# lmmontoya-ai/taboo-brittleness

Measured on AMD Instinct MI355X. Metric: prompts/sec SAE-ablation sweep Gemma-2-9B @L32, higher is better.
Workload: dtype bf16

## Files before the change

taboo_brittleness_amd/csrc/api.h:

```cpp
#pragma once
#include <hip/hip_runtime.h>
#include <stdint.h>

void tb_rmsnorm(const uint16_t* x, const uint16_t* w, uint16_t* y, int M, int D, float eps, hipStream_t st);
void tb_add_rmsnorm2(uint16_t* h, const uint16_t* o, const uint16_t* w_post, const uint16_t* w_next, uint16_t* x,
                     int M, int D, float eps, hipStream_t st);
void tb_embed_rmsnorm(const int32_t* ids, const uint16_t* E, const uint16_t* w, uint16_t* h, uint16_t* x, int M,
                      int D, int V, float scale, float eps, hipStream_t st);
void tb_rope_qkv_cache(const uint16_t* qkv, const int32_t* pos, const int32_t* slot_of_row, const float* cos_t,
                       const float* sin_t, uint16_t* q_out, uint16_t* kc, uint16_t* vc, int M, int Hq, int Hkv,
                       int HD, int S, int max_pos, hipStream_t st);
void tb_rope_qkv_cache_part(const float* part, int ks, const int32_t* pos, const int32_t* slot_of_row,
                            const float* cos_t, const float* sin_t, uint16_t* q_out, uint16_t* kc, uint16_t* vc, int M,
                            int Hq, int Hkv, int HD, int S, int max_pos, hipStream_t st);
void tb_kv_fanout(uint16_t* kc, uint16_t* vc, const int32_t* src_row, const int32_t* slot, const int32_t* pos, int M,
                  int nlayers, int slots, int Hkv, int S, int HD, hipStream_t st);
int tb_attention_lds_bytes(int HD);
int tb_attention_split_rows(int n, bool prefix);
void tb_attention(const uint16_t* q, const uint16_t* kc, const uint16_t* vc, uint16_t* out, const int32_t* pos,
                  const int32_t* slot, int B, int T, int Hq, int Hkv, int HD, int S, float scale, float softcap,
                  int window, hipStream_t st, const uint16_t* pkc = nullptr, const uint16_t* pvc = nullptr,
                  const int32_t* pslot = nullptr, const int32_t* plen = nullptr);
void tb_attention_varlen(const uint16_t* q, const uint16_t* kc, const uint16_t* vc, uint16_t* out, const int32_t* pos,
                         const int32_t* blk, int nblk, int Hq, int Hkv, int HD, int S, float scale, float softcap,
// ... 8 lines not shown
                    int B, int T, int V, int accumulate, int round_bf16, const int32_t* offs, float* cum,
                    const int32_t* rowmap, hipStream_t st);
int tb_topk_chunks(int R, int V);
void tb_topk_rows(const float* x, float* vals, int32_t* idx, int R, int V, int K, float* wv, int32_t* wi, int C,
                  hipStream_t st);
void tb_xent_rows(const uint16_t* logits, const int32_t* tgt, float* nll, int R, int V, float cap, int emulate_bf16,
                  hipStream_t st);
void tb_register_softcap_table(float cap, const uint16_t* tab);
void tb_decode_head(const uint16_t* logits, const int32_t* tgt, int32_t* nxt, float* nll_self, float* nll_tgt, int R,
                    int V, float cap, hipStream_t st);
bool tb_decode_head_stats(const uint16_t* logits, const int32_t* tgt, int off, float* stats, int R, int V, float cap,
                          hipStream_t st);
void tb_head_merge(const float* part, int npart, const int32_t* tgt, const float* tgt_logit, int32_t* nxt,
                   float* nll_self, float* nll_tgt, float* lse, int M, int V, hipStream_t st);
void tb_head_fused4(const uint16_t* A, const uint16_t* W, float* part, float cap, const int32_t* tgt,
                    float* tgt_logit, int32_t* nxt, float* nll_self, float* nll_tgt, int M, int N, int K, hipStream_t st);
void tb_gemm4_qkv_rope(const uint16_t* A, const uint16_t* W, const int32_t* pos, const int32_t* slot_of_row,
                       const uint16_t* cs, uint16_t* q_out, uint16_t* kc, uint16_t* vc, int M, int K,
                       int Hq, int Hkv, int S, int max_pos, int tile_rows, hipStream_t st, const uint16_t* a2 = nullptr,
                       int k0 = 0);
bool tb_register_softcap_compact(float cap, const uint16_t* tab, int lo, int hi, float sat);
bool tb_softcap_compact(const uint16_t* x, float* y, int n, float cap, hipStream_t st);
bool tb_gemm4_ok(int M, int N, int K);
int tb_gemm4_splitk_ks(int M, int N, int K, int tile_rows);
int tb_gemm4_splitk_part(const uint16_t* A, const uint16_t* W, float* ws, int M, int N, int K, int tile_rows, int ks,
                         hipStream_t st);
void tb_add_rmsnorm2_part(uint16_t* h, const float* part, int ks, const uint16_t* w_post, const uint16_t* w_next,
                          uint16_t* x, int M, int D, float eps, hipStream_t st);
void tb_gemm4_splitk(const uint16_t* A, const uint16_t* W, uint16_t* out, float* ws, int M, int N, int K, int ldo,
                     int epi, int tile_rows, int ks, hipStream_t st);
void tb_row_combine(const int64_t* ptr, const float* coef, float* out, int B, int T, int V, hipStream_t st);
bool tb_random_basis_ok(int D);
void tb_random_basis(const uint64_t* seeds, const int32_t* ranks, const int64_t* rows, int n, int D, float* table,
                     hipStream_t st, int qu = 1);
void tb_gemm4(const uint16_t* A, const uint16_t* W, void* C, const float* bias, const float* thr, int M, int N, int K,
              int ldc, int epi, int tile_rows, hipStream_t st, const uint16_t* a2 = nullptr, int k0 = 0);
void tb_gemm_nt(const uint16_t* A, const uint16_t* W, void* C, const float* bias, const float* thr, int M, int N,
                int K, int ldc, int epi, hipStream_t st);
void tb_lowrank_edit(uint16_t* h, uint16_t* x_next, const uint8_t* apply, const int32_t* idx, const int32_t* cnt,
                     int mmax, const void* E, const void* Dm, int table_f32, const float* bias, const float* thr,
                     const float* pre_bias, float alpha, const uint16_t* w_next, float eps, int M, int D,
                     float* coef_out, hipStream_t st, const float* val = nullptr);
void tb_sae_splice_edit(uint16_t* h, uint16_t* x_next, const uint8_t* apply, const int32_t* src_row,
                        const float* acts, int n_act_rows, int L, const int32_t* idx, const int32_t* cnt, int mmax,
                        const void* Wdec, int table_f32, const float* b_dec, float alpha, const uint16_t* w_next,
                        float eps, int M, int D, hipStream_t st);
// ... 61 lines not shown
```

taboo_brittleness_amd/csrc/bindings.cpp:

```cpp
#include <torch/extension.h>
#include <ATen/hip/impl/HIPStreamMasqueradingAsCUDA.h>
#include <c10/core/DeviceGuard.h>

#include <cstdlib>

#include "api.h"

namespace {

hipStream_t cur_stream() { return c10::hip::getCurrentHIPStreamMasqueradingAsCUDA().stream(); }

#define CHECK_DEV(t) TORCH_CHECK((t).is_cuda(), #t " must be a GPU tensor")
#define CHECK_CONTIG(t) TORCH_CHECK((t).is_contiguous(), #t " must be contiguous")
#define CHECK_BF16(t) TORCH_CHECK((t).scalar_type() == at::kBFloat16, #t " must be bfloat16")
#define CHECK_F32(t) TORCH_CHECK((t).scalar_type() == at::kFloat, #t " must be float32")
#define CHECK_I32(t) TORCH_CHECK((t).scalar_type() == at::kInt, #t " must be int32")
#define CHECK_U8(t) TORCH_CHECK((t).scalar_type() == at::kByte || (t).scalar_type() == at::kBool, #t " must be uint8/bool")
#define IN_BF16(t) CHECK_DEV(t); CHECK_CONTIG(t); CHECK_BF16(t)
#define IN_F32(t) CHECK_DEV(t); CHECK_CONTIG(t); CHECK_F32(t)
#define IN_I32(t) CHECK_DEV(t); CHECK_CONTIG(t); CHECK_I32(t)
#define IN_U8(t) CHECK_DEV(t); CHECK_CONTIG(t); CHECK_U8(t)

bool debug_checks() {
  static const bool on = [] {
// ... 369 lines not shown

void gemm4(torch::Tensor A, torch::Tensor W, torch::Tensor C, c10::optional<torch::Tensor> bias,
           c10::optional<torch::Tensor> thr, int64_t epi, int64_t tile_rows) {
  IN_BF16(A); IN_BF16(W); CHECK_DEV(C); CHECK_CONTIG(C);
  TORCH_CHECK(W.dim() == 2, "gemm4: W must be [N, K]");
  TORCH_CHECK(tile_rows == 256 || tile_rows == 128, "gemm4: tile_rows must be 256 or 128");
  const int K = A.size(-1), M = A.numel() / K, N = W.size(0);
  TORCH_CHECK(W.size(1) == K, "gemm4: K mismatch");
  TORCH_CHECK(tb_gemm4_ok(M, N, K), "gemm4: need N % 256 == 0, K % 64 == 0, K >= 64");
  TORCH_CHECK(epi >= 0 && epi <= 3, "gemm4: epi must be 0..3");
  const int64_t ncols = epi == 3 ? N / 2 : N;
  TORCH_CHECK(C.numel() == (int64_t)M * ncols, "gemm4: C shape");
  TORCH_CHECK(C.scalar_type() == ((epi == 0 || epi == 3) ? at::kBFloat16 : at::kFloat), "gemm4: C dtype");
  if (epi == 2) {
    TORCH_CHECK(!bias.has_value() || !bias->defined() || bias->numel() == N, "gemm4: bias numel must be N");
    TORCH_CHECK(!thr.has_value() || !thr->defined() || thr->numel() == N, "gemm4: thr numel must be N");
  }
  c10::DeviceGuard g(A.device());
  tb_gemm4(cbf(A), cbf(W), C.data_ptr(), epi == 2 ? optf(bias) : nullptr, epi == 2 ? optf(thr) : nullptr, M, N, K,
           (int)ncols, (int)epi, (int)tile_rows, cur_stream());
}

bool gemm4_ok(int64_t M, int64_t N, int64_t K) { return tb_gemm4_ok(M, N, K); }

void gemm_ring(torch::Tensor A, torch::Tensor W, torch::Tensor C, int64_t epi, int64_t bm, int64_t bn, int64_t var) {
  IN_BF16(A); IN_BF16(W); IN_BF16(C);
  TORCH_CHECK(W.dim() == 2, "gemm_ring: W must be [N, K]");
  const int K = A.size(-1), M = A.numel() / K, N = W.size(0);
  TORCH_CHECK(W.size(1) == K, "gemm_ring: K mismatch");
  TORCH_CHECK(epi == 0 || epi == 3, "gemm_ring: epi must be 0 or 3");
  TORCH_CHECK(tb_gemm_ring_ok(M, N, K, (int)epi, (int)bm, (int)bn, (int)var), "gemm_ring: unsupported tile / shape");
  const int64_t ncols = epi == 3 ? N / 2 : N;
  TORCH_CHECK(C.numel() == (int64_t)M * ncols, "gemm_ring: C shape");
  c10::DeviceGuard g(A.device());
  tb_gemm_ring(cbf(A), cbf(W), bf(C), M, N, K, (int)ncols, (int)epi, (int)bm, (int)bn, (int)var, cur_stream());
}

bool gemm_ring_ok(int64_t M, int64_t N, int64_t K, int64_t epi, int64_t bm, int64_t bn, int64_t var) {
  return tb_gemm_ring_ok(M, N, K, (int)epi, (int)bm, (int)bn, (int)var);
}

std::vector<std::pair<int64_t, int64_t>> gemm_ring_tiles(int64_t epi) {
  int bm[64], bn[64];
  const int n = std::min(64, tb_gemm_ring_tiles((int)epi, bm, bn, 64));
  std::vector<std::pair<int64_t, int64_t>> out;
  for (int i = 0; i < n; ++i) out.emplace_back(bm[i], bn[i]);
// ... 660 lines not shown
  m.def("row_gather", &row_gather);
  m.def("share_group", &share_group);
  m.def("share_group_max_rows", &share_group_max_rows);
  m.def("attention_split_rows", [](int64_t n, bool prefix) { return (int64_t)tb_attention_split_rows((int)n, prefix); });
  m.def("attention", &attention);
  m.def("attention_prefix", &attention_prefix);
  m.def("attention_varlen", &attention_varlen);
  m.def("attention_varlen_prefix", &attention_varlen_prefix);
  m.def("geglu", &geglu);
  m.def("argmax_rows", &argmax_rows);
  m.def("row_lse", &row_lse);
  m.def("gather_probs", &gather_probs);
  m.def("lens_colsum", &lens_colsum);
  m.def("topk_rows", &topk_rows);
  m.def("xent_rows", &xent_rows);
  m.def("decode_head", &decode_head);
  m.def("decode_head_stats", &decode_head_stats);
  m.def("register_softcap_table", &register_softcap_table);
  m.def("register_softcap_compact", &register_softcap_compact);
  m.def("softcap_compact", &softcap_compact);
  m.def("gemm_nt", &gemm_nt);
  m.def("gemm4", &gemm4);
  m.def("gemm4_ok", &gemm4_ok);
  m.def("gemm_ring", &gemm_ring);
  m.def("gemm_ring_ok", &gemm_ring_ok);
  m.def("gemm_ring_tiles", &gemm_ring_tiles);
  m.def("gemm_ring_qkv_rope", &gemm_ring_qkv_rope);
  m.def("gemm4_splitk", &gemm4_splitk);
  m.def("gemm4_splitk_ks", &gemm4_splitk_ks);
  m.def("gemm4_splitk_part", &gemm4_splitk_part);
  m.def("add_rmsnorm2_part", &add_rmsnorm2_part);
  m.def("gemm4_qkv_rope", &gemm4_qkv_rope);
  m.def("gemm4_l2a", &gemm4_l2a);
  m.def("gemm_ring_l2a", &gemm_ring_l2a);
  m.def("gemm4_qkv_rope_l2a", &gemm4_qkv_rope_l2a);
  m.def("gemm_ring_qkv_rope_l2a", &gemm_ring_qkv_rope_l2a);
  m.def("lora_t", &lora_t);
  m.def("lora_t_chunks", &lora_t_chunks);
  m.def("row_combine", &row_combine);
  m.def("random_basis", &random_basis);
  m.def("lora_t_ok", &lora_t_ok);
  m.def("head_fused", &head_fused);
  m.def("lens_gemm", &lens_gemm);
  m.def("lowrank_edit", &lowrank_edit);
  m.def("latent_affine_edit", &latent_affine_edit);
  m.def("sae_decode_sparse", &sae_decode_sparse);
// ... 21 lines not shown
```

taboo_brittleness_amd/csrc/gemm4.hip:

```cpp
#include "common.h"
#include "api.h"
#include <algorithm>
#include <cstdlib>
#include <utility>

namespace {

constexpr int G4_THREADS = 256, G4_BN = 256;
constexpr int G4_GROUP_M = 4;
constexpr int G4_SLACK1 = 4;
constexpr int G4_SLACK2 = 0;
#ifndef G4_CNT
#define G4_CNT 1
#endif

typedef __attribute__((address_space(3))) void g4_lds_t;
typedef uint32_t u32x2 __attribute__((ext_vector_type(2)));
typedef __attribute__((address_space(3))) char g4_lds_char;

template <int N>
__device__ __forceinline__ void g4_vmcnt() {
  static_assert(N >= 0 && N < 64, "vmcnt range");
  asm volatile("s_waitcnt vmcnt(%0)" ::"n"(N) : "memory");
}
// ... 42 lines not shown

enum { G4_BF16 = 0, G4_F32 = 1, G4_JUMPRELU = 2, G4_GEGLU = 3, G4_ROPE = 4, G4_HEAD = 5, G4_LENS = 6 };

struct G4Rope {
  const int32_t* pos;
  const int32_t* slot;
  const uint16_t* cs;
  uint16_t* q_out;
  uint16_t* kc;
  uint16_t* vc;
  int Hq, Hkv, S, max_pos;
  const uint16_t* ctab;
  int clo, chi;
  float csat, crc, ccap;
  const int32_t* tgt;
  float* tgt_logit;
  float* part;
  int ksplit, kchunk;
  const uint16_t* a2;
  int k0;
};
constexpr int G4_CTAB_N = 32768;

template <int BM, int EPI, bool L2A = false>
__global__ void __launch_bounds__(G4_THREADS, 1)
gemm4_kernel(const uint16_t* __restrict__ A, const uint16_t* __restrict__ W, void* __restrict__ C,
             const float* __restrict__ bias, const float* __restrict__ thr, int M, int N, int K, int ldc, G4Rope rp) {
#if defined(__HIP_DEVICE_COMPILE__)
  static_assert(BM == 256 || BM == 128 || (BM == 64 && EPI == G4_F32), "tile rows (64: the split-K decode tile)");
  constexpr bool G4C = G4_CNT && BM == 256;
  constexpr int WN = 8, WM = BM / 32;
  constexpr int PIMG = G4_BN * 128, QIMG = BM * 128, STG = PIMG + QIMG;
  constexpr int PI = G4_BN / 32, QI = BM / 32, GL = PI + QI;
  constexpr bool LEPI = EPI == G4_BF16 || EPI == G4_LENS;
  constexpr int RB = EPI == G4_GEGLU ? 128 : 256, ECH = RB / 16, ERPI = 64 / ECH;
  constexpr bool SPARE = LEPI;
  constexpr int EXB = SPARE ? 32768 : 0;
  constexpr int ERR = SPARE ? EXB / (4 * RB) : EPI == G4_GEGLU ? BM / 2 : BM / 4;
  constexpr int ENR = LEPI ? (BM / 2) / ERPI : 1;
  constexpr int CTB = EPI == G4_HEAD ? 4096 : 0;
  static_assert(2 * STG + CTB + EXB <= 160 * 1024, "LDS");
  __shared__ __attribute__((aligned(1024))) char smem[2 * STG + CTB + EXB];

  const int nbn = N / G4_BN, nbm = (M + BM - 1) / BM, nwg = nbn * nbm;
  const int NT = K >> 6, KS = EPI == G4_F32 && rp.ksplit > 1 ? rp.ksplit : 1, KC = KS > 1 ? rp.kchunk : NT;
  const int nwgv = nwg * KS;
#define G4_TILE(v, m0_, n0_)                                                                              \
  do {                                                                                                    \
    const int q_ = nwgv / 8, r_ = nwgv % 8, x_ = (v) % 8;                                                 \
    int b_ = (x_ < r_ ? x_ * (q_ + 1) : r_ * (q_ + 1) + (x_ - r_) * q_) + (v) / 8;                        \
    sk = b_ / nwg;                                                                                        \
    b_ -= sk * nwg;                                                                                       \
// ... 17 lines not shown
  for (int i = 0; i < PI; ++i) vp[i] = (uint32_t)((8 * (4 * i + wid) + (lane >> 3)) * K + lchunk * 8) * 2u;
  int mrows, abytes, abytes2 = 0, nt;
  void *wtile, *atile, *atile2 = nullptr;
#define G4_DESC()                                                                                 \
  do {                                                                                            \
    mrows = min(BM, M - m0);                                                                      \
    wtile = (void*)(W + (size_t)n0 * K + sk * KC * 64);                                           \
    atile = (void*)(A + (size_t)m0 * KA + sk * KC * 64);                                          \
    nt = min(KC, NT - sk * KC);                                                                   \
    abytes = mrows * KA * 2;                                                                      \
    int ln_ = __builtin_amdgcn_mbcnt_hi(~0u, __builtin_amdgcn_mbcnt_lo(~0u, 0u));    \
    asm volatile("" : "+v"(ln_));                                                                 \
    const int lc_ = (ln_ & 7) ^ ((4 * wid + (ln_ >> 4)) & 7);                                     \
    _Pragma("unroll") for (int i = 0; i < QI; ++i)                                                \
      vq[i] = (uint32_t)(min(8 * (4 * i + wid) + (ln_ >> 3), mrows - 1) * KA + lc_ * 8) * 2u;     \
    if constexpr (L2A) {                                                                          \
      atile2 = (void*)(rp.a2 + (size_t)m0 * K2);                                                  \
      abytes2 = mrows * K2 * 2;                                                                   \
      _Pragma("unroll") for (int i = 0; i < QI; ++i)                                              \
        vq2[L2A ? i : 0] = (uint32_t)(min(8 * (4 * i + wid) + (ln_ >> 3), mrows - 1) * K2 + lc_ * 8) * 2u; \
    }                                                                                             \
  } while (0)
  G4_DESC();

  const int xr = (lane & 15) >> 1;
  const int co0 = ((lane >> 4) ^ xr) << 4, co1 = ((4 + (lane >> 4)) ^ xr) << 4;
  constexpr bool RP = EPI == G4_ROPE;
  const int offp = (wn * (RP ? 64 : 128) + (lane & 15)) * 128;
#define G4_PROW(i) (RP ? (((i) >> 2) * 128 + ((i) & 3) * 16) : (i) * 16)
  const int offq = PIMG + (wm * (BM / 2) + (lane & 15)) * 128;

  f32x4 acc[WN][WM];
#pragma unroll
  for (int i = 0; i < WN; ++i)
#pragma unroll
    for (int j = 0; j < WM; ++j) acc[i][j] = (f32x4){0.f, 0.f, 0.f, 0.f};
  bf16x8 p0[WN], q0[WM], p1[WN], q1[WM];

  auto frag = [&](int stg, int off) {
    return __builtin_bit_cast(bf16x8, *reinterpret_cast<const uint4*>(smem + stg * STG + off));
  };
#define G4_STAGE_ONE(g, t, stg)                                                                                    \
  do {                                                                                                             \
    char* d_ = smem + (stg) * STG + wid * 1024;                                                                    \
    if ((g) < PI)                                                                                                  \
      __builtin_amdgcn_raw_ptr_buffer_load_lds(__builtin_amdgcn_make_buffer_rsrc(wtile, 0, wbytes, 0x00020000),    \
                                               (g4_lds_t*)(d_ + (g) * 4096), 16, vp[(g) < PI ? (g) : 0], (t) * 128, 0, 0); \
    else if constexpr (L2A) {                 \
      const bool s2_ = (t) >= NT0;                                                                                 \
      __builtin_amdgcn_raw_ptr_buffer_load_lds(                                                                    \
          __builtin_amdgcn_make_buffer_rsrc(s2_ ? atile2 : atile, 0, s2_ ? abytes2 : abytes, 0x00020000),          \
          (g4_lds_t*)(d_ + PIMG + ((g) - PI) * 4096), 16,                                                          \
          s2_ ? vq2[(g) >= PI ? (g) - PI : 0] : vq[(g) >= PI ? (g) - PI : 0], s2_ ? ((t) - NT0) * 128 : (t) * 128,  \
          0, 0);                                                                                                   \
    } else                                                                                                         \
      __builtin_amdgcn_raw_ptr_buffer_load_lds(__builtin_amdgcn_make_buffer_rsrc(atile, 0, abytes, 0x00020000),    \
                                               (g4_lds_t*)(d_ + PIMG + ((g) - PI) * 4096), 16,                      \
                                               vq[(g) >= PI ? (g) - PI : 0], (t) * 128, 0, 0);                      \
  } while (0)
#define G4_STAGE(t, stg) _Pragma("unroll") for (int g_ = 0; g_ < GL; ++g_) G4_STAGE_ONE(g_, t, stg)
#define G4_MFMA(i, j, pc, qc) asm volatile("v_mfma_f32_16x16x32_bf16 %0, %1, %2, %0" : "+a"(acc[i][j]) : "v"(pc[i]), "v"(qc[j]))
#define G4_MF(u)                                                          \
  do {                                                                    \
    if ((u) < NMF) G4_MFMA((u) / WM, (u) % WM, p0, q0);                   \
    else G4_MFMA(((u) - NMF) / WM, ((u) - NMF) % WM, p1, q1);             \
  } while (0)
  constexpr int NR = WN + WM, NMF = WN * WM, NT2 = 2 * NMF;
  constexpr int BAR1 = NR + G4_SLACK1;
  constexpr int BAR2 = NT2 - NR - G4_SLACK2;
  constexpr int GSP = (NT2 - BAR1) / GL;
  constexpr int N2S = (BAR2 - BAR1) / GSP < GL ? (BAR2 - BAR1) / GSP : GL;
  constexpr int N2 = N2S;
  static_assert(GSP >= 1 && BAR1 < NMF && BAR1 < BAR2, "schedule");
  static_assert(NR - 2 <= 15 && BAR1 >= NR, "lgkmcnt range");
#define G4_PK(i) (G4_PROW(i) / 16)
#define G4_QK(j) (PIMG / 2048 + (j))
#define G4_WAIT()                                                        \
  do {                                                                   \
    if (G4C) asm volatile("s_waitcnt lgkmcnt(%0)" ::"n"(NR - 2));     \
  } while (0)
  const uint32_t lds0 = (uint32_t)(uintptr_t)((g4_lds_char*)smem);
  const uint32_t bp0 = lds0 + offp + co0, bp1 = lds0 + offp + co1;
  const uint32_t bq0 = lds0 + offq - PIMG + co0, bq1 = lds0 + offq - PIMG + co1;

  if constexpr (EPI == G4_HEAD) {
    if (rp.ctab != nullptr) {
      uint16_t* lt = reinterpret_cast<uint16_t*>(smem + 2 * STG);
      for (int i = tid; i < rp.chi - rp.clo; i += G4_THREADS) lt[i] = rp.ctab[i];
    }
    __syncthreads();
  }
  G4_STAGE(0, 0);
  G4_STAGE(min(1, nt - 1), 1);
  bool first_tile = true;
  for (;;) {
  if (first_tile || !LEPI) g4_vmcnt<GL>();
  else g4_vmcnt<GL + ENR>();
  first_tile = false;
  g4_bar();
  if (G4C) {
    asm volatile("s_waitcnt lgkmcnt(0)" ::: "memory");
    g4_rd(p0[0], bp0, G4_PK(0));
#pragma unroll
    for (int j = 0; j < WM; ++j) g4_rd(q0[j], bq0, G4_QK(j));
#pragma unroll
    for (int i = 1; i < WN; ++i) g4_rd(p0[i], bp0, G4_PK(i));
  } else {
#pragma unroll
    for (int i = 0; i < WN; ++i) p0[i] = frag(0, offp + G4_PROW(i) * 128 + co0);
#pragma unroll
    for (int j = 0; j < WM; ++j) q0[j] = frag(0, offq + j * 2048 + co0);
  }

#define G4_POST(u)                                                                              \
  do {                                                                                          \
    if ((u) == BAR2) {                                                                          \
      __builtin_amdgcn_s_waitcnt(g4_vmcnt_enc(N2));                                             \
      g4_bar();                                                                                 \
    }                                                                                           \
    G4_MF(u);                                                                                   \
    const int v_ = (u) - BAR2;                                                                  \
    if (v_ >= 0 && v_ < NR) {                                                                   \
      if (G4C) {                                                                             \
        const uint32_t o_ = (sb ^ 1) * STG;                                                     \
        if (v_ == 0) g4_rd(p0[0], bp0 + o_, G4_PK(0));                                          \
        else if (v_ <= WM) g4_rd(q0[v_ >= 1 && v_ <= WM ? v_ - 1 : 0], bq0 + o_, G4_QK(v_ - 1)); \
        else g4_rd(p0[v_ > WM && v_ < NR ? v_ - WM : 0], bp0 + o_, G4_PK(v_ - WM));             \
      } else if (v_ < WN) p0[v_ >= 0 && v_ < WN ? v_ : 0] = frag(sb ^ 1, offp + G4_PROW(v_) * 128 + co0); \
      else q0[v_ >= WN && v_ < NR ? v_ - WN : 0] = frag(sb ^ 1, offq + (v_ - WN) * 2048 + co0); \
    }                                                                                           \
  } while (0)

  for (int t = 0; t < nt; ++t) {
    const int sb = t & 1, tn = min(t + 2, nt - 1);
#pragma unroll
    for (int u = 0; u < NR; ++u) {
      G4_WAIT();
      G4_MF(u);
      if (G4C) {
        if (u < WN) g4_rd(p1[u < WN ? u : 0], bp1 + sb * STG, G4_PK(u));
        else g4_rd(q1[u >= WN ? u - WN : 0], bq1 + sb * STG, G4_QK(u - WN));
      } else if (u < WN) p1[u < WN ? u : 0] = frag(sb, offp + G4_PROW(u) * 128 + co1);
      else q1[u >= WN ? u - WN : 0] = frag(sb, offq + (u - WN) * 2048 + co1);
    }
#pragma unroll
    for (int u = NR; u < BAR1; ++u) {
      G4_WAIT();
      G4_MF(u);
    }
    __builtin_amdgcn_s_waitcnt(0xc07f);
    g4_bar();
#pragma unroll
    for (int g = 0; g < GL; ++g) {
#pragma unroll
      for (int k = 0; k < GSP; ++k) G4_POST(BAR1 + g * GSP + k);
      G4_STAGE_ONE(g, tn, sb);
    }
#pragma unroll
    for (int u = BAR1 + GL * GSP; u < NT2; ++u) G4_POST(u);
    if (!G4C) asm volatile("s_waitcnt lgkmcnt(0)" ::: "memory");
    __builtin_amdgcn_sched_barrier(0);
  }
  if (G4C) asm volatile("s_waitcnt lgkmcnt(0)" ::: "memory");
#undef G4_WAIT
#undef G4_POST
#undef G4_MF
#undef G4_MFMA
  g4_vmcnt<0>();
  g4_bar();
  const int em0 = m0, en0 = n0, esk = sk;
  const int next = tile + (int)gridDim.x;
  if constexpr (LEPI) {
    if (next < nwgv) {
      tile = next;
      G4_TILE(tile, m0, n0);
      G4_DESC();
      G4_STAGE(0, 0);
      if constexpr (SPARE) G4_STAGE(min(1, nt - 1), 1);
    }
    asm volatile("s_nop 15\n\ts_nop 15" ::: "memory");
    const uint32_t reg = (uint32_t)(uintptr_t)((g4_lds_char*)smem) + (SPARE ? 2 * STG + CTB : STG) + wid * ERR * RB;
    uint16_t* obase = reinterpret_cast<uint16_t*>(C) + (size_t)(em0 + wm * (BM / 2)) * ldc;
    const int nrow = min(BM / 2, M - em0 - wm * (BM / 2));
    const auto ors = __builtin_amdgcn_make_buffer_rsrc(obase, 0, nrow > 0 ? nrow * ldc * 2 : 0, 0x00020000);
    int ln = __builtin_amdgcn_mbcnt_hi(~0u, __builtin_amdgcn_mbcnt_lo(~0u, 0u));
    asm volatile("" : "+v"(ln));
    const int oc0 = (EPI == G4_GEGLU ? (en0 >> 1) + wn * 64 : en0 + wn * 128) + (ln % ECH) * 8;
    constexpr int NI = EPI == G4_GEGLU ? WN / 2 : WN, NRA = ECH / ERPI;
    uint32_t wa[NI], ra[NRA];
#pragma unroll
    for (int i = 0; i < NI; ++i) {
      const int cb = 32 * i + 8 * (ln >> 4);
      wa[i] = reg + (ln & 15) * RB + (((cb >> 4) ^ (ln & 15 & (ECH - 1))) << 4) + (cb & 15);
    }
// ... 224 lines not shown
      const int n = nb + i * 16;
      float4 bn_ = make_float4(0.f, 0.f, 0.f, 0.f), th = bn_;
      if constexpr (EPI == G4_JUMPRELU) {
        if (bias) bn_ = *reinterpret_cast<const float4*>(bias + n);
        if (thr) th = *reinterpret_cast<const float4*>(thr + n);
      }
#pragma unroll
      for (int j = 0; j < WM; ++j) {
        const int m = mb + j * 16;
        if (m >= M) continue;
        const f32x4 v = acc[i][j];
        if constexpr (EPI == G4_F32) {
          *reinterpret_cast<float4*>(reinterpret_cast<float*>(C) + ((size_t)esk * M + m) * ldc + n) =
              make_float4(v[0], v[1], v[2], v[3]);
        } else {
          const float a0 = v[0] + bn_.x, a1 = v[1] + bn_.y, a2 = v[2] + bn_.z, a3 = v[3] + bn_.w;
          *reinterpret_cast<float4*>(reinterpret_cast<float*>(C) + (size_t)m * ldc + n) =
              make_float4(a0 > th.x ? a0 : 0.f, a1 > th.y ? a1 : 0.f, a2 > th.z ? a2 : 0.f, a3 > th.w ? a3 : 0.f);
        }
      }
    }
  }
  }
  if (next >= nwgv) break;
#pragma unroll
  for (int i = 0; i < WN; ++i)
#pragma unroll
    for (int j = 0; j < WM; ++j) acc[i][j] = (f32x4){0.f, 0.f, 0.f, 0.f};
  }
  g4_vmcnt<0>();
#undef G4_STAGE
#undef G4_STAGE_ONE
#undef G4_TILE
#undef G4_DESC
#endif
}

template <int EPI>
__global__ void __launch_bounds__(256) g4_splitk_reduce_kernel(const float* __restrict__ part, uint16_t* __restrict__ out,
                                                               int M, int N, int ks, int ldo) {
  const int nout = EPI == G4_GEGLU ? N / 2 : N;
  const size_t i = (size_t)blockIdx.x * blockDim.x + threadIdx.x;
  const int per_row = nout / 8;
  if (i >= (size_t)M * per_row) return;
  const int m = (int)(i / per_row), c8 = (int)(i % per_row) * 8;
  const size_t plane = (size_t)M * N;
  float o[8];
  if constexpr (EPI == G4_GEGLU) {
    const int blk = c8 >> 6, fi = c8 & 63;
    const float* g = part + (size_t)m * N + blk * 128 + fi;
    float gs[8], us[8];
    for (int e = 0; e < 8; ++e) gs[e] = us[e] = 0.f;
    sum_splits8(g, plane, ks, gs);
    sum_splits8(g + 64, plane, ks, us);
    for (int e = 0; e < 8; ++e) o[e] = rbf(gelu_tanh_fast(rbf(gs[e]))) * rbf(us[e]);
  } else {
    for (int e = 0; e < 8; ++e) o[e] = 0.f;
    sum_splits8(part + (size_t)m * N + c8, plane, ks, o);
  }
  *reinterpret_cast<uint4*>(out + (size_t)m * ldo + c8) =
      make_uint4(pack2(o[0], o[1]), pack2(o[2], o[3]), pack2(o[4], o[5]), pack2(o[6], o[7]));
}

}

namespace {
int g4_grid(int nwg) {
  static const int cap = [] {
    int dev = 0, cus = 256;
    if (hipGetDevice(&dev) == hipSuccess) (void)hipDeviceGetAttribute(&cus, hipDeviceAttributeMultiprocessorCount, dev);
    return std::max(8, cus - cus % 8);
  }();
  return std::min(nwg, cap);
}
}

bool tb_gemm4_ok(int M, int N, int K) { return M > 0 && N > 0 && N % G4_BN == 0 && K >= 64 && K % 64 == 0; }

void tb_gemm4(const uint16_t* A, const uint16_t* W, void* C, const float* bias, const float* thr, int M, int N, int K,
              int ldc, int epi, int tile_rows, hipStream_t st, const uint16_t* a2, int k0) {
  if (M <= 0 || N <= 0) return;
  G4Rope rp{};
#define G4_GO(BM_, E_)                                                                                          \
  hipLaunchKernelGGL((gemm4_kernel<BM_, E_>), dim3(g4_grid((N / G4_BN) * ((M + (BM_) - 1) / (BM_)))),            \
                     dim3(G4_THREADS), 0, st, A, W, C, bias, thr, M, N, K, ldc, rp)
#define G4_GO2(BM_, E_)                                                                                         \
  hipLaunchKernelGGL((gemm4_kernel<BM_, E_, true>), dim3(g4_grid((N / G4_BN) * ((M + (BM_) - 1) / (BM_)))),      \
                     dim3(G4_THREADS), 0, st, A, W, C, bias, thr, M, N, K, ldc, rp)
#define G4_EPI(BM_)                                   \
  switch (epi) {                                      \
    case G4_BF16: G4_GO(BM_, G4_BF16); break;         \
    case G4_F32: G4_GO(BM_, G4_F32); break;           \
    case G4_JUMPRELU: G4_GO(BM_, G4_JUMPRELU); break; \
    default: G4_GO(BM_, G4_GEGLU);                    \
  }
  if (a2 != nullptr) {
    rp.a2 = a2;
    rp.k0 = k0;
    if (tile_rows == 128) {
      if (epi == G4_GEGLU) G4_GO2(128, G4_GEGLU);
      else G4_GO2(128, G4_BF16);
    } else {
      if (epi == G4_GEGLU) G4_GO2(256, G4_GEGLU);
      else G4_GO2(256, G4_BF16);
    }
    return;
  }
  if (tile_rows == 128) {
    G4_EPI(128)
  } else {
    G4_EPI(256)
  }
#undef G4_EPI
}

int tb_gemm4_splitk_ks(int M, int N, int K, int tile_rows) {
  const int nwg = (N / G4_BN) * ((M + tile_rows - 1) / tile_rows), NT = K / 64;
  int ks = std::max(1, std::min(g4_grid(1 << 30) / std::max(nwg, 1), NT / 4));
  const int kc = (NT + ks - 1) / ks;
  return (NT + kc - 1) / kc;
}

int tb_gemm4_splitk_part(const uint16_t* A, const uint16_t* W, float* ws, int M, int N, int K, int tile_rows, int ks,
                         hipStream_t st) {
  const int NT = K / 64;
  ks = std::max(1, std::min(ks, NT));
  const int kc = (NT + ks - 1) / ks;
  ks = (NT + kc - 1) / kc;
  if (M <= 0 || N <= 0) return ks;
  G4Rope rp{};
  rp.ksplit = ks;
  rp.kchunk = kc;
// ... 45 lines not shown
    rp.csat = sat;
    rp.crc = 1.0f / cap;
    rp.ccap = cap;
  } else {
    rp.clo = 0x7f81;
    rp.chi = 0x7f82;
    rp.crc = rp.ccap = 1.f;
  }
  rp.tgt = tgt;
  rp.tgt_logit = tgt_logit;
  G4_GO(256, G4_HEAD);
  tb_head_merge(reinterpret_cast<const float*>(part), N / 128, tgt, tgt_logit, nxt, nll_self, nll_tgt, nullptr, M, N, st);
}

void tb_lens_gemm4(const uint16_t* A, const uint16_t* W, uint16_t* logits, float* part, float* lse, int M, int N,
                   int K, hipStream_t st) {
  if (M <= 0) return;
  void* C = logits;
  const float* bias = nullptr;
  const float* thr = nullptr;
  const int ldc = N;
  G4Rope rp{};
  rp.part = part;
  G4_GO(256, G4_LENS);
  tb_head_merge(part, N / 128, nullptr, nullptr, nullptr, nullptr, nullptr, lse, M, N, st);
}

void tb_gemm4_qkv_rope(const uint16_t* A, const uint16_t* W, const int32_t* pos, const int32_t* slot_of_row,
                       const uint16_t* cs, uint16_t* q_out, uint16_t* kc, uint16_t* vc, int M, int K,
                       int Hq, int Hkv, int S, int max_pos, int tile_rows, hipStream_t st, const uint16_t* a2, int k0) {
  if (M <= 0) return;
  const int N = (Hq + 2 * Hkv) * 256, ldc = 0;
  void* C = nullptr;
  const float* bias = nullptr;
  const float* thr = nullptr;
  G4Rope rp{pos, slot_of_row, cs, q_out, kc, vc, Hq, Hkv, S, max_pos};
  if (a2 != nullptr) {
    rp.a2 = a2;
    rp.k0 = k0;
    if (tile_rows == 128) G4_GO2(128, G4_ROPE);
    else G4_GO2(256, G4_ROPE);
    return;
  }
  if (tile_rows == 128) G4_GO(128, G4_ROPE);
  else G4_GO(256, G4_ROPE);
#undef G4_GO
#undef G4_GO2
}

namespace {

__global__ void __launch_bounds__(256) head_merge_kernel(const float4* __restrict__ part, int npart,
                                                         const int32_t* __restrict__ tgt,
                                                         const float* __restrict__ tgt_logit, int32_t* __restrict__ nxt,
                                                         float* __restrict__ nll_self, float* __restrict__ nll_tgt,
                                                         float* __restrict__ lse_out, int V) {
  __shared__ float sm[4], ss[4];
  __shared__ int si[4];
  const int r = blockIdx.x;
  const float4* p = part + (size_t)r * npart;
  float mx = -INFINITY, s = 0.f;
  int bi = 0x7fffffff;
  auto merge = [&](float m2, float s2, int i2) {
    if (m2 > mx) { s = (mx == -INFINITY ? 0.f : s * __expf(mx - m2)) + s2; mx = m2; bi = i2; }
    else if (m2 == mx) { s += s2; bi = min(bi, i2); }
    else if (m2 != -INFINITY) { s += s2 * __expf(m2 - mx); }
  };
  for (int c = threadIdx.x; c < npart; c += blockDim.x) {
// ... 35 lines not shown
```

taboo_brittleness_amd/isa_check.py:

```python
from __future__ import annotations

import os
import re
import subprocess
import sys
import tempfile
from typing import Dict, List, Set, Tuple

CSRC = os.path.join(os.path.dirname(os.path.abspath(__file__)), "csrc")
HIPCC = os.path.join(os.environ.get("ROCM_PATH", "/opt/rocm"), "bin", "hipcc")

_REG = re.compile(r"\b([va])(?:\[(\d+):(\d+)\]|(\d+)(?!\w))")


def _regs(text: str) -> Set[Tuple[str, int]]:
    out = set()
    for m in _REG.finditer(text):
        kind = m.group(1)
        if m.group(4) is not None:
            out.add((kind, int(m.group(4))))
        else:
            out.update((kind, r) for r in range(int(m.group(2)), int(m.group(3)) + 1))
    return out

# ... 28 lines not shown
                if m:
                    n = int(m.group(1))
                    while len(pending) > n:
                        pending.pop(0)
                continue
            if not op.startswith(("v_", "ds_", "buffer_", "global_", "scratch_")):
                continue
            is_store = op.startswith(("ds_write", "buffer_store", "global_store", "scratch_store"))
            dst = set() if is_store or not ops else _regs(ops[0])
            src = set()
            for o in (ops if is_store else ops[1:]):
                src |= _regs(o)
            if op.startswith("v_mfma"):
                src |= dst
            busy = set().union(*pending) if pending else set()
            hit = (src | dst) & busy
            if hit:
                bad.append(f"pass {rnd} #{k}: {line}  touches outstanding {sorted(hit)[:4]}")
            if op.startswith("ds_"):
                pending.append(dst)
    return bad


def loops(asm: str) -> Dict[str, Tuple[List[str], List[str]]]:
    funcs: Dict[str, List[str]] = {}
    cur = None
    for line in asm.split("\n"):
        m = re.match(r"^(_Z\S+):", line)
        if m:
            cur = m.group(1)
            funcs[cur] = []
            continue
        if cur is not None:
            funcs[cur].append(line)
    out = {}
    for name, body in funcs.items():
        m = re.search(r"gemm4_kernelILi(\d+)ELi(\d+)E", name)
        if not m or m.group(1) != "256":
            continue
        blocks, cur_b = [], []
        for line in body:
            if re.match(r"^\.LBB", line):
                blocks.append(cur_b)
                cur_b = []
            else:
                s = line.strip()
                if s and not s.startswith((";", ".")):
                    cur_b.append(s.split(";")[0].strip())
        blocks.append(cur_b)
        li = max(range(len(blocks)), key=lambda i: sum("mfma" in x for x in blocks[i]))
        pi = li - 1
        while pi >= 0 and not (any(x.startswith("ds_read_b128") for x in blocks[pi]) and
                               not any("mfma" in x for x in blocks[pi])):
            pi -= 1
        pre = [x for b in blocks[max(pi, 0): li] for x in b] if pi >= 0 else []
        out[f"gemm4_kernel<256, {m.group(2)}>"] = (pre, blocks[li])
    return out


def compile_asm(extra=()) -> str:
    with tempfile.TemporaryDirectory() as d:
        src = os.path.join(d, "g4.hip")
        with open(src, "w") as f:
            f.write(f'#include "{os.path.join(CSRC, "gemm4.hip")}"\n'
                    "bool tb_softcap_compact_params(float, const uint16_t**, int*, int*, float*) { return false; }\n")
        out = os.path.join(d, "g4.s")
        subprocess.run([HIPCC, "--offload-arch=gfx950", "-fPIC", "-O3", "-std=c++17", "-munsafe-fp-atomics",
                        "--cuda-device-only", "-S", "-I", CSRC, src, "-o", out] + list(extra), check=True,
                       capture_output=True)
        with open(out) as f:
            return f.read()


def violations(asm: str) -> Dict[str, List[str]]:
    ls = loops(asm)
    out = {k: check_loop(body, pre) + ([] if pre else ["no tile prologue found"]) for k, (pre, body) in ls.items()}
    if not ls:
        out["gemm4_kernel<256, *>"] = ["no 256-row kernel found"]
    return out


def main() -> int:
    ls = loops(compile_asm())
    bad = 0
    for k, (pre, body) in sorted(ls.items()):
        v = check_loop(body, pre)
        if not pre:
            v.append("no tile prologue found")
        nw = sum("lgkmcnt(" in x and "lgkmcnt(0)" not in x for x in body)
        print(f"{k}: {len(body)} instructions, {sum('mfma' in x for x in body)} MFMAs, {nw} counted waits, "
              f"{len(v)} violations")
        for x in v[:5]:
            print("   ", x)
        bad += len(v)
    return 1 if bad or not ls else 0


if __name__ == "__main__":
    sys.exit(main())
```

Measured before the change: 2741.

## Stream next tile's K-slices into LDS during current tile's tail in gemm4

Adds a PIPE variant of the persistent 256-row gemm4 kernel. During the last two K-periods of a tile it prefetches the first two K-slices of the next tile into LDS. It also zeroes the accumulators through the first MFMA (a 0 C-operand) instead of an explicit clear, and skips the inter-tile barrier and fragment reload. The aim is to hide the tile-switch bubble and load latency behind the epilogue. The variant is enabled by default for BF16, GEGLU, LENS and ROPE epilogues when K>=192. It adds buffer-parity bookkeeping and register pinning, which risks races and extra register pressure.

```diff
diff --git a/taboo_brittleness_amd/csrc/api.h b/taboo_brittleness_amd/csrc/api.h
--- a/taboo_brittleness_amd/csrc/api.h
+++ b/taboo_brittleness_amd/csrc/api.h
@@ -54,6 +54,7 @@
 bool tb_register_softcap_compact(float cap, const uint16_t* tab, int lo, int hi, float sat);
 bool tb_softcap_compact(const uint16_t* x, float* y, int n, float cap, hipStream_t st);
 bool tb_gemm4_ok(int M, int N, int K);
+int tb_gemm4_set_pipe(int on);
 int tb_gemm4_splitk_ks(int M, int N, int K, int tile_rows);
 int tb_gemm4_splitk_part(const uint16_t* A, const uint16_t* W, float* ws, int M, int N, int K, int tile_rows, int ks,
                          hipStream_t st);
diff --git a/taboo_brittleness_amd/csrc/bindings.cpp b/taboo_brittleness_amd/csrc/bindings.cpp
--- a/taboo_brittleness_amd/csrc/bindings.cpp
+++ b/taboo_brittleness_amd/csrc/bindings.cpp
@@ -415,6 +415,7 @@
 }
 
 bool gemm4_ok(int64_t M, int64_t N, int64_t K) { return tb_gemm4_ok(M, N, K); }
+int64_t gemm4_set_pipe(int64_t on) { return tb_gemm4_set_pipe((int)on); }
 
 void gemm_ring(torch::Tensor A, torch::Tensor W, torch::Tensor C, int64_t epi, int64_t bm, int64_t bn, int64_t var) {
   IN_BF16(A); IN_BF16(W); IN_BF16(C);
@@ -1121,6 +1122,7 @@
   m.def("gemm_nt", &gemm_nt);
   m.def("gemm4", &gemm4);
   m.def("gemm4_ok", &gemm4_ok);
+  m.def("gemm4_set_pipe", &gemm4_set_pipe);
   m.def("gemm_ring", &gemm_ring);
   m.def("gemm_ring_ok", &gemm_ring_ok);
   m.def("gemm_ring_tiles", &gemm_ring_tiles);
diff --git a/taboo_brittleness_amd/csrc/gemm4.hip b/taboo_brittleness_amd/csrc/gemm4.hip
--- a/taboo_brittleness_amd/csrc/gemm4.hip
+++ b/taboo_brittleness_amd/csrc/gemm4.hip
@@ -88,12 +88,15 @@
 };
 constexpr int G4_CTAB_N = 32768;
 
-template <int BM, int EPI, bool L2A = false>
+template <int BM, int EPI, bool L2A = false, bool PIPE = false>
 __global__ void __launch_bounds__(G4_THREADS, 1)
 gemm4_kernel(const uint16_t* __restrict__ A, const uint16_t* __restrict__ W, void* __restrict__ C,
              const float* __restrict__ bias, const float* __restrict__ thr, int M, int N, int K, int ldc, G4Rope rp) {
 #if defined(__HIP_DEVICE_COMPILE__)
   static_assert(BM == 256 || BM == 128 || (BM == 64 && EPI == G4_F32), "tile rows (64: the split-K decode tile)");
+  static_assert(!PIPE || (BM == 256 && !L2A && (EPI == G4_BF16 || EPI == G4_LENS || EPI == G4_GEGLU || EPI == G4_ROPE)),
+                "cross-tile stream: 256-row tile, one A source, no split-K");
+  static_assert(!PIPE || BM == G4_BN, "PIPE stages A with W's row offsets");
   constexpr bool G4C = G4_CNT && BM == 256;
   constexpr int WN = 8, WM = BM / 32;
   constexpr int PIMG = G4_BN * 128, QIMG = BM * 128, STG = PIMG + QIMG;
@@ -157,6 +160,20 @@
     }                                                                                             \
   } while (0)
   G4_DESC();
+  int par = 0, m0n = 0, n0n = 0, abytes_n = 0;
+  bool has_next = false;
+  void *wtile_n = nullptr, *atile_n = nullptr;
+#define G4_NEXT()                                                                                 \
+  do {                                                                                            \
+    has_next = tile + (int)gridDim.x < nwgv;                                                      \
+    m0n = m0;                                                                                     \
+    n0n = n0;                                                                                     \
+    if (has_next) G4_TILE(tile + (int)gridDim.x, m0n, n0n);                                       \
+    const int mr_ = min(BM, M - m0n);                                                             \
+    wtile_n = (void*)(W + (size_t)n0n * K);                                                       \
+    atile_n = (void*)(A + (size_t)m0n * K);                                                       \
+    abytes_n = mr_ * K * 2;                                                                       \
+  } while (0)
 
   const int xr = (lane & 15) >> 1;
   const int co0 = ((lane >> 4) ^ xr) << 4, co1 = ((4 + (lane >> 4)) ^ xr) << 4;
@@ -166,12 +183,23 @@
   const int offq = PIMG + (wm * (BM / 2) + (lane & 15)) * 128;
 
   f32x4 acc[WN][WM];
-#pragma unroll
-  for (int i = 0; i < WN; ++i)
-#pragma unroll
-    for (int j = 0; j < WM; ++j) acc[i][j] = (f32x4){0.f, 0.f, 0.f, 0.f};
+  if constexpr (!PIPE) {
+#pragma unroll
+    for (int i = 0; i < WN; ++i)
+#pragma unroll
+      for (int j = 0; j < WM; ++j) acc[i][j] = (f32x4){0.f, 0.f, 0.f, 0.f};
+  }
   bf16x8 p0[WN], q0[WM], p1[WN], q1[WM];
 
+#define G4_HOLD_FRAGS()                                                                                          \
+  do {                                                                                                           \
+    asm volatile("s_waitcnt lgkmcnt(0)"                                                                          \
+                 : "+v"(p0[0]), "+v"(p0[1]), "+v"(p0[2]), "+v"(p0[3]), "+v"(p0[4]), "+v"(p0[5]), "+v"(p0[6]),    \
+                   "+v"(p0[7])::"memory");                                                                       \
+    asm volatile("s_waitcnt lgkmcnt(0)"                                                                          \
+                 : "+v"(q0[0]), "+v"(q0[1]), "+v"(q0[2]), "+v"(q0[3]), "+v"(q0[4]), "+v"(q0[5]), "+v"(q0[6]),    \
+                   "+v"(q0[7])::"memory");                                                                       \
+  } while (0)
   auto frag = [&](int stg, int off) {
     return __builtin_bit_cast(bf16x8, *reinterpret_cast<const uint4*>(smem + stg * STG + off));
   };
@@ -193,11 +221,26 @@
                                                (g4_lds_t*)(d_ + PIMG + ((g) - PI) * 4096), 16,                      \
                                                vq[(g) >= PI ? (g) - PI : 0], (t) * 128, 0, 0);                      \
   } while (0)
+#define G4_STAGE_PIPE(g, kt, stg, nx)                                                                              \
+  do {                                                                                                             \
+    char* d_ = smem + (stg) * STG + wid * 1024;                                                                    \
+    if ((g) < PI)                                                                                                  \
+      __builtin_amdgcn_raw_ptr_buffer_load_lds(                                                                    \
+          __builtin_amdgcn_make_buffer_rsrc((nx) ? wtile_n : wtile, 0, wbytes, 0x00020000),                        \
+          (g4_lds_t*)(d_ + (g) * 4096), 16, vp[(g) < PI ? (g) : 0], (kt) * 128, 0, 0);                             \
+    else                                                                                                           \
+      __builtin_amdgcn_raw_ptr_buffer_load_lds(                                                                    \
+          __builtin_amdgcn_make_buffer_rsrc((nx) ? atile_n : atile, 0, (nx) ? abytes_n : abytes, 0x00020000),      \
+          (g4_lds_t*)(d_ + PIMG + ((g) - PI) * 4096), 16,                                                          \
+          vp[(g) >= PI ? (g) - PI : 0], (kt) * 128, 0, 0);                                                         \
+  } while (0)
 #define G4_STAGE(t, stg) _Pragma("unroll") for (int g_ = 0; g_ < GL; ++g_) G4_STAGE_ONE(g_, t, stg)
 #define G4_MFMA(i, j, pc, qc) asm volatile("v_mfma_f32_16x16x32_bf16 %0, %1, %2, %0" : "+a"(acc[i][j]) : "v"(pc[i]), "v"(qc[j]))
+#define G4_MFMA0(i, j, pc, qc) asm volatile("v_mfma_f32_16x16x32_bf16 %0, %1, %2, 0" : "=a"(acc[i][j]) : "v"(pc[i]), "v"(qc[j]))
 #define G4_MF(u)                                                          \
   do {                                                                    \
-    if ((u) < NMF) G4_MFMA((u) / WM, (u) % WM, p0, q0);                   \
+    if ((u) < NMF && zc_) G4_MFMA0((u) / WM, (u) % WM, p0, q0);           \
+    else if ((u) < NMF) G4_MFMA((u) / WM, (u) % WM, p0, q0);              \
     else G4_MFMA(((u) - NMF) / WM, ((u) - NMF) % WM, p1, q1);             \
   } while (0)
   constexpr int NR = WN + WM, NMF = WN * WM, NT2 = 2 * NMF;
@@ -227,24 +270,31 @@
   }
   G4_STAGE(0, 0);
   G4_STAGE(min(1, nt - 1), 1);
+  if constexpr (PIPE) G4_NEXT();
   bool first_tile = true;
   for (;;) {
-  if (first_tile || !LEPI) g4_vmcnt<GL>();
-  else g4_vmcnt<GL + ENR>();
-  first_tile = false;
-  g4_bar();
+  constexpr bool REREAD = PIPE && EPI == G4_ROPE;
+  if (!PIPE || first_tile || REREAD) {
+  if (!PIPE || first_tile) {
+    if (first_tile || !LEPI) g4_vmcnt<GL>();
+    else g4_vmcnt<GL + ENR>();
+    g4_bar();
+  }
   if (G4C) {
     asm volatile("s_waitcnt lgkmcnt(0)" ::: "memory");
-    g4_rd(p0[0], bp0, G4_PK(0));
-#pragma unroll
-    for (int j = 0; j < WM; ++j) g4_rd(q0[j], bq0, G4_QK(j));
-#pragma unroll
-    for (int i = 1; i < WN; ++i) g4_rd(p0[i], bp0, G4_PK(i));
+    const uint32_t o_ = par * STG;
+    g4_rd(p0[0], bp0 + o_, G4_PK(0));
+#pragma unroll
+    for (int j = 0; j < WM; ++j) g4_rd(q0[j], bq0 + o_, G4_QK(j));
+#pragma unroll
+    for (int i = 1; i < WN; ++i) g4_rd(p0[i], bp0 + o_, G4_PK(i));
+    if constexpr (PIPE) G4_HOLD_FRAGS();
   } else {
 #pragma unroll
-    for (int i = 0; i < WN; ++i) p0[i] = frag(0, offp + G4_PROW(i) * 128 + co0);
-#pragma unroll
-    for (int j = 0; j < WM; ++j) q0[j] = frag(0, offq + j * 2048 + co0);
+    for (int i = 0; i < WN; ++i) p0[i] = frag(par, offp + G4_PROW(i) * 128 + co0);
+#pragma unroll
+    for (int j = 0; j < WM; ++j) q0[j] = frag(par, offq + j * 2048 + co0);
+  }
   }
 
 #define G4_POST(u)                                                                              \
@@ -255,7 +305,7 @@
     }                                                                                           \
     G4_MF(u);                                                                                   \
     const int v_ = (u) - BAR2;                                                                  \
-    if (v_ >= 0 && v_ < NR) {                                                                   \
+    if (v_ >= 0 && v_ < NR && !noread_) {                                                       \
       if (G4C) {                                                                             \
         const uint32_t o_ = (sb ^ 1) * STG;                                                     \
         if (v_ == 0) g4_rd(p0[0], bp0 + o_, G4_PK(0));                                          \
@@ -266,45 +316,74 @@
     }                                                                                           \
   } while (0)
 
-  for (int t = 0; t < nt; ++t) {
-    const int sb = t & 1, tn = min(t + 2, nt - 1);
-#pragma unroll
-    for (int u = 0; u < NR; ++u) {
-      G4_WAIT();
-      G4_MF(u);
-      if (G4C) {
-        if (u < WN) g4_rd(p1[u < WN ? u : 0], bp1 + sb * STG, G4_PK(u));
-        else g4_rd(q1[u >= WN ? u - WN : 0], bq1 + sb * STG, G4_QK(u - WN));
-      } else if (u < WN) p1[u < WN ? u : 0] = frag(sb, offp + G4_PROW(u) * 128 + co1);
-      else q1[u >= WN ? u - WN : 0] = frag(sb, offq + (u - WN) * 2048 + co1);
-    }
-#pragma unroll
-    for (int u = NR; u < BAR1; ++u) {
-      G4_WAIT();
-      G4_MF(u);
-    }
-    __builtin_amdgcn_s_waitcnt(0xc07f);
-    g4_bar();
-#pragma unroll
-    for (int g = 0; g < GL; ++g) {
-#pragma unroll
-      for (int k = 0; k < GSP; ++k) G4_POST(BAR1 + g * GSP + k);
-      G4_STAGE_ONE(g, tn, sb);
-    }
-#pragma unroll
-    for (int u = BAR1 + GL * GSP; u < NT2; ++u) G4_POST(u);
-    if (!G4C) asm volatile("s_waitcnt lgkmcnt(0)" ::: "memory");
-    __builtin_amdgcn_sched_barrier(0);
-  }
+  first_tile = false;
+#define G4_PERIOD(t, tn, nx, lastp, zc)                                                            \
+  do {                                                                                             \
+    constexpr bool zc_ = (zc);        \
+    const int sb = ((t) + par) & 1;                                                                \
+    constexpr bool noread_ = REREAD && (lastp);    \
+    _Pragma("unroll") for (int u = 0; u < NR; ++u) {       \
+      G4_WAIT();                                                                                   \
+      G4_MF(u);                                                                                    \
+      if (G4C) {                                                                                   \
+        if (u < WN) g4_rd(p1[u < WN ? u : 0], bp1 + sb * STG, G4_PK(u));                           \
+        else g4_rd(q1[u >= WN ? u - WN : 0], bq1 + sb * STG, G4_QK(u - WN));                       \
+      } else if (u < WN) p1[u < WN ? u : 0] = frag(sb, offp + G4_PROW(u) * 128 + co1);             \
+      else q1[u >= WN ? u - WN : 0] = frag(sb, offq + (u - WN) * 2048 + co1);                      \
+    }                                                                                              \
+    _Pragma("unroll") for (int u = NR; u < BAR1; ++u) {                                            \
+      G4_WAIT();                                                                                   \
+      G4_MF(u);                                                                                    \
+    }                                                                                              \
+    __builtin_amdgcn_s_waitcnt(0xc07f);                                                            \
+    g4_bar();                                                                                      \
+    _Pragma("unroll") for (int g = 0; g < GL; ++g) {                                               \
+      _Pragma("unroll") for (int k = 0; k < GSP; ++k) G4_POST(BAR1 + g * GSP + k);                 \
+      if constexpr (PIPE) G4_STAGE_PIPE(g, tn, sb, nx);                                            \
+      else G4_STAGE_ONE(g, tn, sb);                                                                \
+    }                                                                                              \
+    _Pragma("unroll") for (int u = BAR1 + GL * GSP; u < NT2; ++u) G4_POST(u);                      \
+    if (!G4C) asm volatile("s_waitcnt lgkmcnt(0)" ::: "memory");                                   \
+    __builtin_amdgcn_sched_barrier(0);                                                             \
+  } while (0)
+  if constexpr (!PIPE) {
+    for (int t = 0; t < nt; ++t) {
+      const int tn = min(t + 2, nt - 1);
+      G4_PERIOD(t, tn, false, false, false);
+    }
+  } else {
+    G4_PERIOD(0, 2, false, false, true);
+    for (int t = 1; t < nt - 2; ++t) G4_PERIOD(t, t + 2, false, false, false);
+    const int kt0 = __builtin_amdgcn_readfirstlane(has_next ? 0 : nt - 1);
+    const int kt1 = __builtin_amdgcn_readfirstlane(has_next ? 1 : nt - 1);
+    G4_PERIOD(nt - 2, kt0, true, false, false);
+    G4_PERIOD(nt - 1, kt1, true, true, false);
+  }
+#undef G4_PERIOD
   if (G4C) asm volatile("s_waitcnt lgkmcnt(0)" ::: "memory");
 #undef G4_WAIT
 #undef G4_POST
 #undef G4_MF
 #undef G4_MFMA
-  g4_vmcnt<0>();
-  g4_bar();
+#undef G4_MFMA0
+  if constexpr (!PIPE) {
+    g4_vmcnt<0>();
+    g4_bar();
+  } else if (G4C && !REREAD) {
+    G4_HOLD_FRAGS();
+  }
   const int em0 = m0, en0 = n0, esk = sk;
-  const int next = tile + (int)gridDim.x;
+  const int next = PIPE ? nwgv : tile + (int)gridDim.x;
+  const bool more = PIPE ? has_next : next < nwgv;
+  if constexpr (PIPE) {
+    tile += (int)gridDim.x;
+    m0 = m0n;
+    n0 = n0n;
+    wtile = wtile_n;
+    atile = atile_n;
+    abytes = abytes_n;
+    par ^= nt & 1;
+  }
   if constexpr (LEPI) {
     if (next < nwgv) {
       tile = next;
@@ -575,15 +654,22 @@
     }
   }
   }
-  if (next >= nwgv) break;
-#pragma unroll
-  for (int i = 0; i < WN; ++i)
-#pragma unroll
-    for (int j = 0; j < WM; ++j) acc[i][j] = (f32x4){0.f, 0.f, 0.f, 0.f};
+  if (!more) break;
+  if constexpr (PIPE) {
+    G4_NEXT();
+  } else {
+#pragma unroll
+    for (int i = 0; i < WN; ++i)
+#pragma unroll
+      for (int j = 0; j < WM; ++j) acc[i][j] = (f32x4){0.f, 0.f, 0.f, 0.f};
+  }
   }
   g4_vmcnt<0>();
 #undef G4_STAGE
 #undef G4_STAGE_ONE
+#undef G4_HOLD_FRAGS
+#undef G4_STAGE_PIPE
+#undef G4_NEXT
 #undef G4_TILE
 #undef G4_DESC
 #endif
@@ -626,7 +712,10 @@
   }();
   return std::min(nwg, cap);
 }
-}
+int g4_pipe = 1;
+}
+
+int tb_gemm4_set_pipe(int on) { return std::exchange(g4_pipe, on != 0); }
 
 bool tb_gemm4_ok(int M, int N, int K) { return M > 0 && N > 0 && N % G4_BN == 0 && K >= 64 && K % 64 == 0; }
 
@@ -640,6 +729,13 @@
 #define G4_GO2(BM_, E_)                                                                                         \
   hipLaunchKernelGGL((gemm4_kernel<BM_, E_, true>), dim3(g4_grid((N / G4_BN) * ((M + (BM_) - 1) / (BM_)))),      \
                      dim3(G4_THREADS), 0, st, A, W, C, bias, thr, M, N, K, ldc, rp)
+#define G4_GOP(E_)                                                                                              \
+  do {                                                                                                          \
+    if (g4_pipe && K >= 192)                                                                                    \
+      hipLaunchKernelGGL((gemm4_kernel<256, E_, false, true>), dim3(g4_grid((N / G4_BN) * ((M + 255) / 256))),   \
+                         dim3(G4_THREADS), 0, st, A, W, C, bias, thr, M, N, K, ldc, rp);                         \
+    else G4_GO(256, E_);                                                                                        \
+  } while (0)
 #define G4_EPI(BM_)                                   \
   switch (epi) {                                      \
     case G4_BF16: G4_GO(BM_, G4_BF16); break;         \
@@ -661,6 +757,10 @@
   }
   if (tile_rows == 128) {
     G4_EPI(128)
+  } else if (epi == G4_BF16) {
+    G4_GOP(G4_BF16);
+  } else if (epi == G4_GEGLU) {
+    G4_GOP(G4_GEGLU);
   } else {
     G4_EPI(256)
   }
@@ -752,7 +852,7 @@
   const int ldc = N;
   G4Rope rp{};
   rp.part = part;
-  G4_GO(256, G4_LENS);
+  G4_GOP(G4_LENS);
   tb_head_merge(part, N / 128, nullptr, nullptr, nullptr, nullptr, nullptr, lse, M, N, st);
 }
 
@@ -773,7 +873,8 @@
     return;
   }
   if (tile_rows == 128) G4_GO(128, G4_ROPE);
-  else G4_GO(256, G4_ROPE);
+  else G4_GOP(G4_ROPE);
+#undef G4_GOP
 #undef G4_GO
 #undef G4_GO2
 }
diff --git a/taboo_brittleness_amd/isa_check.py b/taboo_brittleness_amd/isa_check.py
--- a/taboo_brittleness_amd/isa_check.py
+++ b/taboo_brittleness_amd/isa_check.py
@@ -74,7 +74,7 @@
     return bad
 
 
-def loops(asm: str) -> Dict[str, Tuple[List[str], List[str]]]:
+def loops(asm: str, variants: bool = False) -> Dict[str, Tuple[List[str], List[str]]]:
     funcs: Dict[str, List[str]] = {}
     cur = None
     for line in asm.split("\n"):
@@ -87,27 +87,56 @@
             funcs[cur].append(line)
     out = {}
     for name, body in funcs.items():
-        m = re.search(r"gemm4_kernelILi(\d+)ELi(\d+)E", name)
+        m = re.search(r"gemm4_kernelILi(\d+)ELi(\d+)E(?:Lb([01])ELb([01])E)?", name)
         if not m or m.group(1) != "256":
             continue
-        blocks, cur_b = [], []
+        blocks, cur_b, labels = [], [], [""]
         for line in body:
             if re.match(r"^\.LBB", line):
                 blocks.append(cur_b)
                 cur_b = []
+                labels.append(line.split(":")[0])
             else:
                 s = line.strip()
                 if s and not s.startswith((";", ".")):
                     cur_b.append(s.split(";")[0].strip())
         blocks.append(cur_b)
-        li = max(range(len(blocks)), key=lambda i: sum("mfma" in x for x in blocks[i]))
+        nmf = [sum("mfma" in x for x in b) for b in blocks]
+        pipe = m.group(4) == "1"
+        if pipe:
+            li = next(i for i, n in enumerate(nmf) if n >= 100 and any(
+                x.startswith("s_cbranch") and x.split()[-1] == labels[i] for x in blocks[i]))
+            ti = next((i for i in range(li + 1, len(blocks)) if nmf[i] >= 200), None)
+        else:
+            li = max(range(len(blocks)), key=lambda i: nmf[i])
+            ti = li + 1 if li + 1 < len(blocks) else None
+        def _top(blk):
+            fm = next((i for i, x in enumerate(blk) if "mfma" in x), len(blk))
+            nrd = sum(x.startswith("ds_read_b128") for x in blk[:fm])
+            return nrd > 0 and (fm == len(blk) or (pipe and nrd >= 16))
+
         pi = li - 1
-        while pi >= 0 and not (any(x.startswith("ds_read_b128") for x in blocks[pi]) and
-                               not any("mfma" in x for x in blocks[pi])):
+        while pi >= 0 and not _top(blocks[pi]):
             pi -= 1
         pre = [x for b in blocks[max(pi, 0): li] for x in b] if pi >= 0 else []
-        out[f"gemm4_kernel<256, {m.group(2)}>"] = (pre, blocks[li])
+        key = f"gemm4_kernel<256, {m.group(2)}>"
+        if variants:
+            key = f"gemm4_kernel<256, {m.group(2)}, {m.group(3) or 0}, {m.group(4) or 0}>"
+        elif key in out and (pipe or m.group(3) == "1"):
+            continue
+        out[key] = (pre, blocks[li])
+        tail = []
+        if ti is not None:
+            last = max([i for i, x in enumerate(blocks[ti]) if "mfma" in x], default=-1)
+            for i, x in enumerate(blocks[ti]):
+                tail.append(x)
+                if i > last and x.startswith("s_waitcnt") and "lgkmcnt(0)" in x:
+                    break
+        _TAILS[key] = tail
     return out
+
+
+_TAILS: Dict[str, List[str]] = {}
 
 
 def compile_asm(extra=()) -> str:
@@ -124,19 +153,24 @@
             return f.read()
 
 
+def check_all(key: str, pre: List[str], body: List[str]) -> List[str]:
+    tail = _TAILS.get(key, [])
+    return check_loop(body, pre) + check_loop(tail, body) + check_loop(tail, pre)
+
+
 def violations(asm: str) -> Dict[str, List[str]]:
-    ls = loops(asm)
-    out = {k: check_loop(body, pre) + ([] if pre else ["no tile prologue found"]) for k, (pre, body) in ls.items()}
+    ls = loops(asm, variants=True)
+    out = {k: check_all(k, pre, body) + ([] if pre else ["no tile prologue found"]) for k, (pre, body) in ls.items()}
     if not ls:
         out["gemm4_kernel<256, *>"] = ["no 256-row kernel found"]
     return out
 
 
 def main() -> int:
-    ls = loops(compile_asm())
+    ls = loops(compile_asm(), variants=True)
     bad = 0
     for k, (pre, body) in sorted(ls.items()):
-        v = check_loop(body, pre)
+        v = check_all(k, pre, body)
         if not pre:
             v.append("no tile prologue found")
         nw = sum("lgkmcnt(" in x and "lgkmcnt(0)" not in x for x in body)
```

Result: faster. 2785 (median of 6 runs) (+1.6%).
